# denyingmxd/CFPNet

Measured on AMD Instinct MI355X. Metric: depth maps/sec @ 480x640 bf16 (whole job; per_gpu = value / n_gpus); abs_rel vs CPU oracle, higher is better.
Workload: dtype bf16; 1 GPU; batch=8 480x640 RGB + 8x8-zone ToF, eval forward incl. the prob output [B,256,H/2,W/2] written in the storage dtype (bf16: 2 bytes/element); layers=hist2image combine1 image x2 (CFPNet), parallelism=single GPU

## Files before the change

cfpnet_amd/engine.py:

```python
from __future__ import annotations

import math
import os
from typing import Dict, List, Optional, Sequence, Tuple

import torch

from . import hip, ops, spec
from .geometry import FUSION_SCALES, FusionGeometry, gsa_keys, static_zone_key, zone_records as _zone_records
from .ops import Act

_BN_EPS = 1e-5


def _same_pad(size: int, k: int, s: int) -> Tuple[int, int]:
    total = max((math.ceil(size / s) - 1) * s + k - size, 0)
    return total // 2, total - total // 2


_STREAMS: Dict = {}
_CONCURRENT: Dict[str, list] = {}


def concurrent_streams(device, want: int = 4, pool: int = 16) -> list:
# ... 33 lines not shown
    key = (str(torch.device(device)), role)
    st = _STREAMS.get(key)
    if st is None:
        if isinstance(role, tuple) and role[0] == "lane":
            conc = concurrent_streams(device)
            st = conc[role[1] % len(conc)]
        else:
            st = torch.cuda.Stream(device=device)
        _STREAMS[key] = st
    return st


class Engine:
    def __init__(self, state_dict: Dict[str, torch.Tensor], *, layer_names: Sequence[str], n_bins: int = 256,
                 min_val: float = 1e-3, max_val: float = 10.0, norm: str = "linear", change_embedding: bool = True,
                 no_skip_inside: bool = False, stem_act: bool = False, dtype=None, device="cuda:0",
                 zone_sample_num: int = 16, base_resolution=spec.BASE_RESOLUTION, x3: Optional[bool] = None):
        if dtype is None:
            dtype, x3 = torch.float32, (True if x3 is None else x3)
        x3 = bool(x3)
        hip.load()
        self.base_resolution = tuple(base_resolution)
        self.fusion = spec.fusion_table(self.base_resolution)
        if not torch.cuda.is_available():
            raise RuntimeError("cfpnet_amd.Engine needs a GPU: the product path has no CPU fallback")
        assert dtype in (torch.bfloat16, torch.float16, torch.float32)
        self.layer_names = list(layer_names)
        self.n_bins, self.min_val, self.max_val = n_bins, float(min_val), float(max_val)
        self.norm = {"linear": 0, "softmax": 1, "sigmoid": 2}[norm]
        self.change_embedding, self.no_skip_inside, self.stem_act = change_embedding, no_skip_inside, stem_act
        self.dtype, self.device = dtype, torch.device(device)
        assert not x3 or dtype == torch.float32, "x3 is a matrix-math mode of float32 storage"
        self.x3 = bool(x3)
        self.cdt = hip.F32X3 if self.x3 else ops.DT[dtype]
        self.tickets = self.x3 and os.environ.get("CFP_SPLITK_TICKETS", "0") == "1"
        self.zone_sample_num = zone_sample_num
        self.weights2 = os.environ.get("CFP_WEIGHTS2", "0") == "1"
        self.diffuse_cin = os.environ.get("CFP_DIFFUSE_CIN", "1") == "1"
        self.mbconv_fused = os.environ.get("CFP_MBCONV_FUSED", "0") == "1"
        self.se2 = dtype in (torch.bfloat16, torch.float16) and os.environ.get("CFP_SE2", "1") == "1"
        self.se2_x3 = os.environ.get("CFP_SE2_X3", "1") if self.x3 else "0"
        self._dbg_round = {}
        for item in filter(None, os.environ.get("CFP_DEBUG_ROUND", "").split(",")):
            n, d = item.split(":")
            self._dbg_round[n] = {"f16": torch.float16, "bf16": torch.bfloat16}[d]
        self.up_fused = os.environ.get("CFP_UP_FUSED", "4")
        self.up_fused_x3 = os.environ.get("CFP_UP_FUSED_X3", "")
        self.cat_pad = os.environ.get("CFP_CAT_PAD", "1") == "1" and not self.up_fused_x3
        self.lkpm_fused = os.environ.get("CFP_LKPM_FUSED", "1") != "0"
        self.tail_q = os.environ.get("CFP_TAIL_Q", "1") == "1"
        self.lkpm_min_rows = int(os.environ.get("CFP_LKPM_MIN_ROWS", "30000"))
        self.sr_ln_fused = os.environ.get("CFP_SR_LN_FUSED", "1") == "1"
        self.head_fused = os.environ.get("CFP_HEAD_FUSED", "1") != "0"
        self.er_fused = os.environ.get("CFP_ER_FUSED", "12")
        hl = os.environ.get("CFP_HEAD_HILO", "00")
        self.head_hilo = (hl[0] == "1", hl[1] == "1")
        self.half = dtype in (torch.bfloat16, torch.float16)
        self.ve = 8 if self.half else 4
        self.P: Dict[str, torch.Tensor] = {}
        self._plans: Dict[tuple, dict] = {}
        self._graph = None
        self._splitk_ws: Optional[torch.Tensor] = None
        self._capturing = False
        self._side = _shared_stream(self.device, "side")
        self._lane = 0
        self.use_side_stream = os.environ.get("CFP_NO_SIDE_STREAM", "0") != "1"
        self._lane_streams: Dict[int, Tuple[torch.cuda.Stream, torch.cuda.Stream]] = {}
        self._lanes_active = 1
        self._slots = None
        self._slot_next = 0
        self._lane_ws: Dict[int, torch.Tensor] = {}
        self.load_state_dict(state_dict)

    def _dev(self, t: torch.Tensor, dtype=None) -> torch.Tensor:
        return t.detach().to(device=self.device, dtype=dtype or torch.float32).contiguous()

    def _pack_conv(self, w: torch.Tensor, w2: bool = False) -> torch.Tensor:
        w = w.detach().float()
        if w.dim() == 2:
            w = w[:, :, None, None]
        elif w.dim() == 3:
            w = w[:, :, :, None]
        co, ci, kh, kw = w.shape
        if kh * kw > 1:
            w = ops.round_taps(w, self.dtype)
        cip = (ci + 7) // 8 * 8
        if cip != ci:
            w = torch.nn.functional.pad(w, (0, 0, 0, 0, 0, cip - ci))
        flat = w.permute(0, 2, 3, 1).reshape(co, kh * kw * cip)
        if w2 and self.weights2 and self.half and kh * kw == 1:
            return ops.pack_w2(flat, self.dtype).to(self.device)
        if kh * kw == 1 and self.diffuse_cin and self.dtype == torch.float16:
            flat = ops.round_taps(flat.reshape(co, 1, kh * kw * cip), self.dtype).reshape(co, -1)
        if self.x3:
            return ops.pack_w_x3(self._dev(flat))
        return self._dev(flat, self.dtype)

    def _fold_bn(self, sd, bn: Optional[str], bias: Optional[torch.Tensor], co: int, eps: float):
        if bn is None:
            scale = torch.ones(co)
            shift = bias.detach().float().clone() if bias is not None else torch.zeros(co)
        else:
            g, b = sd[bn + ".weight"].float(), sd[bn + ".bias"].float()
            m, v = sd[bn + ".running_mean"].float(), sd[bn + ".running_var"].float()
            scale = g / torch.sqrt(v + eps)
            shift = b - m * scale
# ... 858 lines not shown
            M = B * hd * wd
            t1 = self._act(plan, f"up{i}.a", M, c[i])
            fits = hd > 1 and wd > 1 and B * hd * wd * cat[i].ld * 2 < 2 ** 31 - 65536 and hs_ * ws_ * src.ld * 2 < 2 ** 31 - 65536
            if self.x3 and str(i) in self.up_fused_x3 and src.C % 32 == 0 and taps is None and hd > 1 and wd > 1:
                n = f"decoder.up{i}.a"
                ops.upsample_cat_conv3x3(src, hs_, ws_, cat[i].slice(src.C, e[i]), self.P[n + ".wcat"], self.P[n + ".s"], self.P[n + ".t"],
                                         t1, B, hd, wd, hip.ACT_LRELU, x3=True)
            elif self.half and str(i) in self.up_fused and src.C % 64 == 0 and taps is None and fits:
                n = f"decoder.up{i}.a"
                ops.upsample_cat_conv3x3(src, hs_, ws_, cat[i].slice(src.C, e[i]), self.P[n + ".w"], self.P[n + ".s"], self.P[n + ".t"],
                                         t1, B, hd, wd, hip.ACT_LRELU)
            else:
                ops.resize_bilinear(src, hs_, ws_, (0, 0, hs_, ws_), cat[i].slice(0, src.C), hd, wd, (0, 0, hd, wd), B)
                n = f"decoder.up{i}.a"
                if (n + ".wpad") in self.P and M >= 30000:
                    ops.conv2d(cat[i], self.P[n + ".wpad"], self.P[n + ".s"], self.P[n + ".t"], t1, B, hd, wd, 3, 3, 1, 1, 1, hd, wd, hip.ACT_LRELU,
                               None, self._ws(M, t1.C, 9 * cat[i].C))
                else:
                    self._cv(n, cat[i].slice(0, src.C + e[i]), t1, B, hd, wd, 3, act=hip.ACT_LRELU)
            if first_only:
                return t1
            t2 = self._act(plan, f"up{i}.b", M, c[i])
            self._cv(f"decoder.up{i}.b", t1, t2, B, hd, wd, 3, act=hip.ACT_LRELU)
            return t2

        main.wait_stream(side)
        xd4 = self._act(plan, "xd4", B * hs[4] * wsz[4], c[0])
        self._cv("decoder.conv4", b4, xd4, B, hs[4], wsz[4], 1)
        x = xd4
        ph, pw = hs[4], wsz[4]
        for i, (fname, feat) in enumerate((("cross_atten3", hfeat[2]), ("cross_atten2", hfeat[1]), ("cross_atten1", hfeat[0])), start=1):
            hh, ww = hs[4 - i], wsz[4 - i]
            D = c[i + 1]
            dcat = self._act(plan, f"dcat{i}", B * hh * ww, 2 * D)
            n3, n1 = f"decoder.up{i}.b", f"decoder.conv{4 - i}"
            if (i == 3 and self.half and (n1 + ".wp") in self.P and "d" in self.er_fused and taps is None
                    and ops.conv3x3_pw_fused_variant(c[i], c[i], D, 1, ops.DT[self.dtype]) >= 0):
                t1 = up(i, x, ph, pw, hh, ww, first_only=True)
                ops.conv3x3_pw_fused(t1, self.P[n3 + ".w"], self.P[n3 + ".s"], self.P[n3 + ".t"], hip.ACT_LRELU, self.P[n1 + ".wp"],
                                     self.P[n1 + ".s"], self.P[n1 + ".t"], dcat.slice(0, D), B, hh, ww, 1, 1, 1, hh, ww)
            else:
                t = up(i, x, ph, pw, hh, ww)
                if taps is not None:
                    taps[f"up{i}"] = self._nchw(t, B, hh, ww)
                self._cv(n1, t, dcat.slice(0, D), B, hh, ww, 1)
            fuse(fname, dcat.slice(0, D), feat, hh, ww, dcat.slice(D, D))
            if taps is not None:
                taps[f"conv{4 - i}"] = self._nchw(dcat.slice(0, D), B, hh, ww)
                taps[fname] = self._nchw(dcat.slice(D, D), B, hh, ww)
            x, ph, pw = dcat, hh, ww
        t = up(4, x, ph, pw, hs[0], wsz[0])
        Mh = B * hs[0] * wsz[0]
        HWh = hs[0] * wsz[0]
        unet = self._act(plan, "unet", Mh, 128)
        fused_head = self.half and self.head_fused and self.n_bins == 256 and HWh % 16 == 0 and HWh >= 128 and "conv_out.wp" in self.P
        ram = self._act(plan, "ram", Mh, 128) if (not fused_head or taps is not None) else None
        edges = out[0] if out is not None else torch.empty(B, self.n_bins + 1, dtype=torch.float32, device=dev)
        centers = self._f32(plan, "head.centers", B * self.n_bins)
        h = "depth_head"
        ns = max(1, min(64, HWh // 256))
        bsum = self._f32(plan, "head.bsum", B * ns * t.C)
        msum = self._f32(plan, "head.msum", B * 128)
        if os.environ.get("CFP_OLD_SUMS", "0") == "1":
            self._cv("decoder.conv0", t, unet, B, hs[0], wsz[0], 3)
        side.wait_stream(main)
        with torch.cuda.stream(side):
            ops.channel_sum(t, bsum, B, HWh, ns)
            ops.conv3x3_mean(bsum, ns, t, self.P["decoder.conv0.w32"], self.P["decoder.conv0.b32"], msum, B, hs[0], wsz[0], 128)
            ops.bin_regressor(msum, 1, 1.0 / HWh, self.P[h + ".w1x1"], self.P[h + ".r0.w"], self.P[h + ".r0.b"], self.P[h + ".r2.w"],
                              self.P[h + ".r2.b"], self.P[h + ".r4.w"], self.P[h + ".r4.b"], self.min_val, self.max_val, self.norm,
                              edges, centers, B, 128, 256, self.n_bins)
        if os.environ.get("CFP_OLD_SUMS", "0") != "1":
            self._cv("decoder.conv0", t, unet, B, hs[0], wsz[0], 3)
        if not fused_head:
            self._cv("depth_head.conv3x3", unet, ram, B, hs[0], wsz[0], 3)
        main.wait_stream(side)
        pred = out[1] if out is not None else torch.empty(B, 1, hs[0], wsz[0], dtype=torch.float32, device=dev)
        if out is not None:
            prob = out[2] if return_prob else None
        else:
            prob = torch.empty(B, self.n_bins, hs[0], wsz[0], dtype=self.dtype, device=dev) if return_prob else None
        unc = None
        if uncertainty:
            unc = out[3] if out is not None else torch.empty(B, 3, hs[0], wsz[0], dtype=torch.float32, device=dev)
        if fused_head:
            ops.depth_head_fused(unet, self.P[h + ".conv3x3.w"], self.P[h + ".conv3x3.s"], self.P[h + ".conv3x3.t"], self.P["conv_out.wp"],
                                 self.P["conv_out.t"], centers, prob, pred, B, hs[0], wsz[0], ram_out=ram, ram_hilo=self.head_hilo[1],
                                 stats=unc)
        elif (self.half or self.x3) and self.n_bins == 256 and HWh % 8 == 0 and os.environ.get("CFP_BIN_HEAD_FUSED", "1") != "0":
            ops.bin_head_fused(ram, self.P["conv_out.w"], self.P["conv_out.t"], centers, prob, pred, B, HWh, stats=unc)
        else:
            logits = self._act(plan, "logits", Mh, self.n_bins)
            self._lin("conv_out.w", ram, logits, Mh, hip.ACT_NONE, None, "conv_out")
            ops.bin_softmax(logits, centers, prob, pred, B, HWh, self.n_bins, stats=unc)
        if taps is not None:
            taps["unet_out"] = self._nchw(unet, B, hs[0], wsz[0])
            taps["ram"] = self._nchw(ram, B, hs[0], wsz[0])
        return (edges, pred, prob, unc) if uncertainty else (edges, pred, prob)
```

cfpnet_amd/hip.py:

```python
from __future__ import annotations

import ctypes as C
import os
from typing import Optional

_HERE = os.path.dirname(os.path.abspath(__file__))
LIB_PATH = os.environ.get("CFP_HIP_LIB") or os.path.join(_HERE, "libcfpnet_hip.so")

F32, BF16, F16 = 0, 1, 2
F32X3 = 3
ACT_NONE, ACT_RELU, ACT_LRELU, ACT_SILU, ACT_GELU, ACT_SIGMOID = range(6)
TOF_SAMPLE_UNIFORM, TOF_SAMPLE_ICDF = 0, 1
HEAD_WOUT_HILO, HEAD_RAM_HILO = 1, 2
UNC_STD, UNC_ENTROPY, UNC_PMAX = 0, 1, 2
SPARS_STD, SPARS_ENTROPY, SPARS_PMAX, SPARS_ORACLE_RMSE, SPARS_ORACLE_ABSREL = range(5)
REGION_ALL, REGION_FOV_IN, REGION_FOV_OUT, REGION_ZONE_VALID, REGION_ZONE_INVALID = range(5)
CONV_PER_IMAGE, CONV_W2, CONV_IN_FLIGHT, CONV_X3, CONV_WS_TICKETS = 1, 2, 4, 8, 16
CONV_TICKET_BYTES = 4096

_p, _i, _f, _sz, _ll = C.c_void_p, C.c_int, C.c_float, C.c_size_t, C.c_longlong

SIGNATURES = {
    "cfp_version": (_i, []),
    "cfp_last_error": (C.c_char_p, []),
# ... 80 lines not shown
    "cfp_bn_train_bwd": (_i, [_p, _i, _p, _i, C.c_longlong, _i, _i, _p, _p, _p, _p, _i, _p, _p, _p, _i, _p, _sz, _p]),
    "cfp_colsum": (_i, [_p, _i, C.c_longlong, _i, _i, _p, _p, _sz, _p]),
    "cfp_act_bwd": (_i, [_p, _i, _p, _i, _i, _p, _i, C.c_longlong, _i, _i, _p]),
    "cfp_layernorm_bwd_ws_bytes": (_sz, [C.c_longlong, _i]),
    "cfp_layernorm_bwd": (_i, [_p, _i, _p, _i, _p, _f, _p, _i, _i, _p, _p, C.c_longlong, _i, _i, _p, _sz, _p]),
    "cfp_layernorm_bwd_deferred": (_i, [_p, _i, _p, _i, _p, _f, _p, _i, _i, _p, _p, C.c_longlong, _i, _i, _p, _sz, _p, _p]),
    "cfp_axpby": (_i, [_p, _i, _p, _i, _f, _f, _p, _i, C.c_longlong, _i, _i, _p]),
    "cfp_rowtable_grad": (_i, [_p, _i, _p, _i, _i, _i, _i, _i, _i, _i, _f, _i, _p]),
    "cfp_se_train_ws_floats": (_sz, [_i, _i, _i]),
    "cfp_se_train_fwd": (_i, [_p, _i, _f] + [_p] * 7 + [_i, _i, _i, _p]),
    "cfp_se_train_bwd": (_i, [_p] * 12 + [_f, _f, _i, _i, _i, _p]),
    "cfp_channel_dot": (_i, [_p, _i, _p, _i, _p, _i, _i, _i, _i, _p]),
    "cfp_bcast_fma": (_i, [_p, _i, _p, _p, _p, _i, _i, _i, _i, _i, _p]),
    "cfp_dwconv3x3_dgrad": (_i, [_p, _i, _p, _p, _i] + [_i] * 11 + [_p]),
    "cfp_dwconv3x3_wgrad_ws_bytes": (_sz, [_i]),
    "cfp_dwconv3x3_wgrad": (_i, [_p, _i, _p, _i, _p] + [_i] * 9 + [_f, _i, _p, _sz, _p]),
    "cfp_dwconv3x3_wgrad_deferred": (_i, [_p, _i, _p, _i, _p] + [_i] * 9 + [_f, _i, _p, _sz, _p, _p]),
    "cfp_index_rows": (_i, [_p, _i, _p, _p, _i, C.c_longlong, _i, _i, _i, _p]),
    "cfp_resize_bilinear_bwd": (_i, [_p, _i, _p, _i, _i, _i, _i, _i, _i, _i, _i, _i, _p]),
    "cfp_bin_centers": (_i, [_p, _f, _f, _p, _p, _i, _i, _p]),
    "cfp_bin_centers_bwd": (_i, [_p, _f, _f, _p, _i, _i, _p]),
    "cfp_softmax_expect_ws_bytes": (_sz, [_i, _i, _i]),
    "cfp_softmax_expect": (_i, [_p, _i, _p, _p, _p, _p, _i, _p, _i, _i, _i, _i, _p, _sz, _p]),
    "cfp_linattn_state_bytes": (_sz, [_i, _i, _i]),
    "cfp_linattn_ws_bytes": (_sz, [_i, _i, _i, _i, _i]),
    "cfp_linattn_fwd": (_i, [_p, _i, _p, _i, _p, _i, _p, _i, _p, _i, _i, _i, _i, _i, _f, _i, _p, _sz, _p]),
    "cfp_linattn_bwd": (_i, [_p, _i, _p, _i, _p, _i, _p, _i, _p, _p, _i, _p, _i, _p, _i, _i, _i, _i, _i, _i, _f, _i, _p, _sz, _p]),
    "cfp_linattn_fwd_dev": (_i, [_p, _i, _p, _i, _p, _i, _p, _i, _p, _i, _i, _i, _i, _i, _f, _i, _p, _sz, _p, _p]),
    "cfp_linattn_bwd_dev": (_i, [_p, _i, _p, _i, _p, _i, _p, _i, _p, _p, _i, _p, _i, _p, _i, _i, _i, _i, _i, _i, _f, _i, _p, _sz, _p, _p]),
    "cfp_zone_crop": (_i, [_p, _i, _p, _p, _i] + [_i] * 7 + [_i, _p]),
    "cfp_zone_crop_bwd": (_i, [_p, _i, _p, _p, _i] + [_i] * 7 + [_i, _p]),
    "cfp_zone_paste": (_i, [_p, _i, _p, _i, _p, _p, _i] + [_i] * 7 + [_i, _p]),
    "cfp_zone_paste_bwd": (_i, [_p, _i, _p, _p, _i] + [_i] * 7 + [_i, _p]),
    "cfp_zone_rect_rows": (_i, [_p, _i, _p, _p, _i] + [_i] * 6 + [_i, _p]),
    "cfp_dwconv_large_wgrad_ws_bytes": (_sz, [_i, _i, _i, _i, _i]),
    "cfp_dwconv_large_wgrad": (_i, [_p, _i, _p, _i, _p, _i, _i, _i, _i, _i, _f, _i, _p, _sz, _p]),
    "cfp_row_normalize": (_i, [_p, _p, _p, _i, _i, _p]),
    "cfp_add_rowtable_dev": (_i, [_p, _i, _p, _p, _i, _i, _i, _i, _i, _i, _i, _p, _i, _p]),
    "cfp_rowtable_grad_dev": (_i, [_p, _i, _p, _i, _i, _i, _i, _i, _i, _p, _f, _i, _p]),
    "cfp_nyu_augment": (_i, [_p, _p, _i, _i, _i, _p, _p, _p, _i, _i, C.POINTER(C.c_float), C.POINTER(C.c_float), _p, _p, _p]),
    "cfp_nyu_rotate": (_i, [_p, _p, _p, _p, _i, _i, _i, _p, _p]),
    "cfp_bin_regressor": (_i, [_p, _i, _f] + [_p] * 7 + [_f, _f, _i, _p, _p, _i, _i, _i, _i, _p]),
    "cfp_bin_softmax": (_i, [_p, _i, _p, _p, _p, _i, _i, _i, _i, _p]),
    "cfp_bin_softmax_stats": (_i, [_p, _i, _p, _p, _p, _p, _i, _i, _i, _i, _p]),
    "cfp_conv3x3_mean": (_i, [_p, _i, _p, _i, _p, _p, _p, _i, _i, _i, _i, _i, _i, _p]),
    "cfp_lkpm_tail": (_i, [_p, _i, _p, _i, _p, _i, _p, _p, _p, _p, _p, _p, _f, _i, _i, _i, _p]),
    "cfp_mbconv_plan": (_i, [_i, _i, _i, _i, _i, _p, _p]),
    "cfp_mbconv_expand_dw": (_i, [_p, _i, _p, _p, _p, _p, _p, _p, _p, _i, _p, _i, _i, _i, _i, _i, _i, _p]),
    "cfp_conv3x3_pw_fused_variant": (_i, [_i] * 5),
    "cfp_conv3x3_pw_fused": (_i, [_p, _i, _p, _p, _p, _i, _p, _p, _p, _i, _p, _i, _p, _i] + [_i] * 12 + [_p]),
    "cfp_hist_encoder": (_i, [_p, _p, _p, _p, _p, _p, _p, _p, _p, _i, _i, _i, _p]),
    "cfp_depth_head_fused": (_i, [_p, _i, _p, _p, _p, _p, _p, _p, _p, _p, _p, _i, _i, _i, _i, _i, _p]),
    "cfp_bin_head_fused": (_i, [_p, _i, _p, _p, _p, _p, _p, _i, _i, _i, _i, _p]),
    "cfp_depth_head_fused_stats": (_i, [_p, _i, _p, _p, _p, _p, _p, _p, _p, _p, _p, _p, _i, _i, _i, _i, _i, _p]),
    "cfp_bin_head_fused_stats": (_i, [_p, _i, _p, _p, _p, _p, _p, _p, _i, _i, _i, _i, _p]),
}

class WgradJob(C.Structure):
    _fields_ = [("slabs", C.c_void_p), ("dw", C.c_void_p), ("db", C.c_void_p), ("n", C.c_longlong), ("n_dw", C.c_longlong),
                ("nsplit", C.c_int), ("ew", C.c_int), ("beta", C.c_float), ("beta_b", C.c_float)]


_lib: Optional[C.CDLL] = None


def load() -> C.CDLL:
    global _lib
    if _lib is not None:
        return _lib
    if not os.path.exists(LIB_PATH):
        raise RuntimeError(
            f"{LIB_PATH} not found: build the HIP extension first "
            f"(`python -c 'import __graft_entry__ as g; g.build()'` or `make -C cfpnet_amd/csrc`). "
            "There is no CPU fallback for the product path.")
    import torch
    lib = C.CDLL(LIB_PATH)
    for name, (res, args) in SIGNATURES.items():
        fn = getattr(lib, name)
        fn.restype = res
        fn.argtypes = args
    _lib = lib
    return lib


def last_error() -> str:
    return load().cfp_last_error().decode()


def call(name: str, *args):
    rc = getattr(load(), name)(*args)
    if rc != 0:
        raise RuntimeError(f"{name} failed ({rc}): {last_error()}")


def ptr(t) -> int:
    return 0 if t is None else t.data_ptr()


def current_stream() -> int:
    import torch
    return torch.cuda.current_stream().cuda_stream
```

cfpnet_amd/ops.py:

```python
from __future__ import annotations

import os
from dataclasses import dataclass
from typing import Optional, Tuple

import torch

from . import hip

DT = {torch.float32: hip.F32, torch.bfloat16: hip.BF16, torch.float16: hip.F16}


@dataclass
class Act:
    buf: torch.Tensor
    c0: int
    C: int

    @property
    def rows(self) -> int:
        return self.buf.shape[0]

    @property
    def ld(self) -> int:
# ... 453 lines not shown
    wp = w[:, src]
    hi = (round_taps(w.reshape(256, 1, 128), dtype).reshape(256, 128)[:, src] if diffuse else wp).to(dtype)
    planes = [hi]
    if hilo:
        planes.append((wp - hi.float()).to(dtype))
    return torch.stack(planes).contiguous()


def pw_k_order(K: int) -> torch.Tensor:
    pos = torch.arange((K + 31) // 32 * 32)
    kb, q, e = pos // 32, (pos % 32) // 8, pos % 8
    src = 32 * kb + 16 * (e // 4) + 4 * q + (e % 4)
    return torch.where(src < K, src, torch.full_like(src, -1))


def pad_pw_w(w: torch.Tensor) -> torch.Tensor:
    co, K = w.shape
    out = torch.zeros((co + 15) // 16 * 16, (K + 31) // 32 * 32, dtype=w.dtype, device=w.device)
    out[:co, :K] = w
    return out.contiguous()


def conv3x3_pw_fused_variant(Cin: int, Cmid: int, Cout: int, stride: int, dt: int) -> int:
    return int(hip.load().cfp_conv3x3_pw_fused_variant(Cin, Cmid, Cout, stride, dt))


def conv3x3_pw_fused(x: Act, w1: torch.Tensor, s1, t1, act1, w2_pad: torch.Tensor, s2, t2, out: Act, B, H, W, stride, pad_t, pad_l, Ho, Wo,
                     act2=hip.ACT_NONE, residual: Optional[Act] = None):
    mid = w1.shape[0]
    assert x.rows >= B * H * W and out.rows >= B * Ho * Wo and x.dt == out.dt
    assert w1.dtype == x.buf.dtype and tuple(w1.shape) == (mid, 9 * x.C) and w1.is_contiguous()
    assert w2_pad.dtype == x.buf.dtype and tuple(w2_pad.shape) == ((out.C + 15) // 16 * 16, (mid + 31) // 32 * 32) and w2_pad.is_contiguous()
    hip.call("cfp_conv3x3_pw_fused", x.ptr, x.ld, w1.data_ptr(), hip.ptr(s1), hip.ptr(t1), act1, w2_pad.data_ptr(), hip.ptr(s2), hip.ptr(t2), act2,
             residual.ptr if residual else 0, residual.ld if residual else 0, out.ptr, out.ld, B, H, W, x.C, mid, out.C, stride, pad_t, pad_l,
             Ho, Wo, x.dt, _s())


def depth_head_fused(x: Act, w3, scale3, shift3, wout_perm: torch.Tensor, bias_out, centers, prob, pred, B, H, W, ram_out: Optional[Act] = None,
                     ram_hilo: bool = True, probe: int = 0, stats=None):
    assert x.C == 128 and w3.shape == (128, 9 * 128) and wout_perm.shape[1:] == (256, 128) and wout_perm.dtype == x.buf.dtype
    flags = (hip.HEAD_WOUT_HILO if wout_perm.shape[0] == 2 else 0) | (hip.HEAD_RAM_HILO if ram_hilo else 0) | (probe << 8)
    if ram_out is not None:
        assert ram_out.ld == 128 and ram_out.C == 128
    if stats is None:
        hip.call("cfp_depth_head_fused", x.ptr, x.ld, w3.data_ptr(), hip.ptr(scale3), hip.ptr(shift3), wout_perm.data_ptr(), bias_out.data_ptr(),
                 centers.data_ptr(), hip.ptr(prob), pred.data_ptr(), ram_out.ptr if ram_out is not None else 0, B, H, W, flags, x.dt, _s())
        return
    _check_stats(stats, B, H * W)
    hip.call("cfp_depth_head_fused_stats", x.ptr, x.ld, w3.data_ptr(), hip.ptr(scale3), hip.ptr(shift3), wout_perm.data_ptr(), bias_out.data_ptr(),
             centers.data_ptr(), hip.ptr(prob), pred.data_ptr(), stats.data_ptr(), ram_out.ptr if ram_out is not None else 0, B, H, W, flags,
             x.dt, _s())


def hist_encoder(hist: torch.Tensor, blob: torch.Tensor, layout, outs, R: int, pe=(None, None, None), n_pe: int = 0):
    import ctypes
    assert hist.dtype == torch.float32 and hist.is_contiguous() and hist.numel() >= R and blob.dtype == torch.float32 and len(layout) == 9
    flat = [int(v) for row in layout for v in row]
    arr = (ctypes.c_int * len(flat))(*flat)
    for o, row in zip(outs, layout[2::3]):
        assert o.C == row[4] and o.ld == o.C and o.c0 == 0 and o.rows >= R
    for t, o in zip(pe, outs):
        assert t is None or (t.dtype == torch.float32 and tuple(t.shape) == (n_pe, o.C) and t.is_contiguous())
    hip.call("cfp_hist_encoder", hist.data_ptr(), blob.data_ptr(), ctypes.addressof(arr), outs[0].ptr, outs[1].ptr, outs[2].ptr,
             hip.ptr(pe[0]), hip.ptr(pe[1]), hip.ptr(pe[2]), n_pe, R, outs[0].dt, _s())


def conv3x3_mean(partial: torch.Tensor, nsplit, x: Act, w32: torch.Tensor, bias, msum: torch.Tensor, B, H, W, Cout):
    assert w32.dtype == torch.float32 and tuple(w32.shape) == (Cout, 9 * x.C) and msum.dtype == torch.float32 and msum.numel() >= B * Cout
    hip.call("cfp_conv3x3_mean", partial.data_ptr(), nsplit, x.ptr, x.ld, w32.data_ptr(), hip.ptr(bias), msum.data_ptr(), B, H, W, x.C, Cout, x.dt, _s())


def mbconv_plan(B, H, W, Cin, mid):
    import ctypes
    t, kp = ctypes.c_int(0), ctypes.c_int(0)
    rc = hip.load().cfp_mbconv_plan(B, H, W, Cin, mid, ctypes.byref(t), ctypes.byref(kp))
    return (t.value, kp.value) if rc == 0 else None


def pack_mbconv_pw(w2d: torch.Tensor, dtype) -> torch.Tensor:
    mid, cin = w2d.shape
    kp = (cin + 31) // 32 * 32
    out = torch.zeros(mid, kp + 8, dtype=dtype)
    out[:, :cin] = w2d.to(dtype)
    return out.contiguous()


def mbconv_expand_dw(x: Act, wpw: torch.Tensor, s1, t1, wdw: torch.Tensor, s2, t2, out: Act, partial: Optional[torch.Tensor], B, H, W):
    mid = out.C
    assert wpw.dtype == x.buf.dtype and wpw.shape[0] == mid and wdw.shape == (9, mid) and wdw.dtype == x.buf.dtype
    hip.call("cfp_mbconv_expand_dw", x.ptr, x.ld, wpw.data_ptr(), s1.data_ptr(), t1.data_ptr(), wdw.data_ptr(), s2.data_ptr(), t2.data_ptr(),
             out.ptr, out.ld, hip.ptr(partial), B, H, W, x.C, mid, x.dt, _s())


def lkpm_tail(t: Act, xin: Act, out: Act, w1, b1, w2, b2, ln_g, ln_b, rows, ln_eps=1e-6):
    D = t.C
    x3 = t.buf.dtype == torch.float32 and w1.dtype == torch.float16
    k1, k2 = (2 * D, 8 * D) if x3 else (D, 4 * D)
    assert xin.C == D and out.C == D and tuple(w1.shape) == (4 * D, k1) and tuple(w2.shape) == (D, k2) and (x3 or w1.dtype == t.buf.dtype)
    hip.call("cfp_lkpm_tail", t.ptr, t.ld, xin.ptr, xin.ld, out.ptr, out.ld, w1.data_ptr(), b1.data_ptr(), w2.data_ptr(), b2.data_ptr(),
             ln_g.data_ptr(), ln_b.data_ptr(), float(ln_eps), rows, D, hip.F32X3 if x3 else t.dt, _s())
```

include/cfpnet_hip.h:

```cpp
#ifndef CFPNET_HIP_H
#define CFPNET_HIP_H

#include <stddef.h>
#include <stdint.h>

#ifdef __cplusplus
extern "C" {
#endif

typedef void* cfp_stream_t;

enum { CFP_OK = 0, CFP_EINVAL = -1, CFP_ESHAPE = -2, CFP_EHIP = -3 };
enum { CFP_F32 = 0, CFP_BF16 = 1, CFP_F16 = 2 };
enum { CFP_F32X3 = 3 };
enum { CFP_TOF_SAMPLE_UNIFORM = 0, CFP_TOF_SAMPLE_ICDF = 1 };
enum { CFP_ACT_NONE = 0, CFP_ACT_RELU = 1, CFP_ACT_LRELU = 2, CFP_ACT_SILU = 3, CFP_ACT_GELU = 4, CFP_ACT_SIGMOID = 5 };

int cfp_version(void);
const char* cfp_last_error(void);

int cfp_conv2d_nhwc(const void* in, int in_ld, const void* w, const float* scale, const float* shift,
                    const void* residual, int res_ld, void* out, int out_ld,
                    int B, int H, int W, int Cin, int Cout, int KH, int KW, int stride,
                    int pad_t, int pad_l, int Ho, int Wo, int act, int dtype,
// ... 107 lines not shown
int cfp_resize_bilinear(const void* src, int src_ld, int Hs, int Ws, int sy0, int sx0, int sh, int sw,
                        void* dst, int dst_ld, int Hd, int Wd, int dy0, int dx0, int dh, int dw,
                        const uint8_t* zone_valid, int zn, int p1, int p2, int accumulate,
                        int B, int C, int dtype, cfp_stream_t stream);

int cfp_resize_bilinear_dev(const void* src, int src_ld, int Hs, int Ws, void* dst, int dst_ld, int Hd, int Wd,
                            const int* rec, int rec_side, const uint8_t* zone_valid, int zn, int p1, int p2,
                            int accumulate, int B, int C, int dtype, cfp_stream_t stream);

int cfp_add_rowtable(const void* in, int in_ld, const float* table, void* out, int out_ld, int rows, int C,
                     int H, int W, int Wt, int oy, int ox, int dtype, cfp_stream_t stream);

int cfp_upsample_cat_conv3x3(const void* low, int low_ld, int Hs, int Ws, int Cup, const void* skip, int skip_ld, int Cskip,
                             const void* w, const float* scale, const float* shift, void* out, int out_ld, int B, int H, int W,
                             int Cout, int act, int dtype, cfp_stream_t stream);

int cfp_copy_rows(const void* in, int in_ld, void* out, int out_ld, int rows, int C, int dtype, cfp_stream_t stream);
int cfp_copy_rows2(const void* in0, int in0_ld, void* out0, int out0_ld, int C0, const void* in1, int in1_ld, void* out1, int out1_ld,
                   int C1, int rows, int dtype, cfp_stream_t stream);

int cfp_rgb_to_nhwc8(const float* rgb, void* out, int B, int H, int W, int dtype, cfp_stream_t stream);
int cfp_rgb_to_nhwc8_hilo(const float* rgb, void* out, int B, int H, int W, int dtype, cfp_stream_t stream);
int cfp_scalar_to_rows8(const float* in, void* out, int rows, int dtype, cfp_stream_t stream);

int cfp_hist_encoder(const float* hist, const float* blob, const int* layout, void* out0, void* out1, void* out2,
                     const float* pe0, const float* pe1, const float* pe2, int n_pe, int R, int dtype, cfp_stream_t stream);

int cfp_lkpm_tail(const void* t, int t_ld, const void* xin, int x_ld, void* out, int out_ld, const void* w1, const float* b1,
                  const void* w2, const float* b2, const float* ln_g, const float* ln_b, float ln_eps, int rows, int D, int dtype,
                  cfp_stream_t stream);

int cfp_bin_regressor(const float* partial, int nsplit, float inv_hw, const float* w1x1_t,
                      const float* w0_t, const float* b0, const float* w1_t, const float* b1,
                      const float* w2_t, const float* b2, float min_val, float max_val, int norm,
                      float* edges, float* centers, int B, int C, int hidden, int nbins, cfp_stream_t stream);

int cfp_conv3x3_mean(const float* partial, int nsplit, const void* in, int in_ld, const float* w, const float* bias, float* msum,
                     int B, int H, int W, int C, int Cout, int dtype, cfp_stream_t stream);

int cfp_bin_softmax(const void* logits, int ld, const float* centers, void* prob, float* pred,
                    int B, int HW, int nbins, int dtype, cfp_stream_t stream);

enum { CFP_UNC_STD = 0, CFP_UNC_ENTROPY = 1, CFP_UNC_PMAX = 2 };
int cfp_bin_softmax_stats(const void* logits, int ld, const float* centers, void* prob, float* pred, float* stats,
                          int B, int HW, int nbins, int dtype, cfp_stream_t stream);

enum { CFP_HEAD_WOUT_HILO = 1, CFP_HEAD_RAM_HILO = 2 };
int cfp_depth_head_fused(const void* x, int x_ld, const void* w3, const float* scale3, const float* shift3,
                         const void* wout_perm, const float* bias_out, const float* centers, void* prob, float* pred,
                         void* ram_out, int B, int H, int W, int flags, int dtype, cfp_stream_t stream);
int cfp_depth_head_fused_stats(const void* x, int x_ld, const void* w3, const float* scale3, const float* shift3,
                               const void* wout_perm, const float* bias_out, const float* centers, void* prob, float* pred,
                               float* stats, void* ram_out, int B, int H, int W, int flags, int dtype, cfp_stream_t stream);

int cfp_bin_head_fused(const void* x, int x_ld, const void* w, const float* bias, const float* centers,
                       void* prob, float* pred, int B, int HW, int Cin, int dtype, cfp_stream_t stream);
int cfp_bin_head_fused_stats(const void* x, int x_ld, const void* w, const float* bias, const float* centers,
                             void* prob, float* pred, float* stats, int B, int HW, int Cin, int dtype, cfp_stream_t stream);


size_t cfp_silog_ws_bytes(int B, int Ht, int Wt);
int cfp_silog_loss_fwd(const float* pred, int Hp, int Wp, const float* target, const unsigned char* mask, int Ht, int Wt,
                       int B, int interpolate, void* ws, size_t ws_bytes, float* stats, cfp_stream_t stream);
int cfp_silog_loss_bwd(const void* ws, const float* stats, float grad_loss, int Hp, int Wp, int Ht, int Wt, int B,
                       int interpolate, float* grad_pred, cfp_stream_t stream);

int cfp_adamw_step(float* param, const float* grad, float* exp_avg, float* exp_avg_sq, long long n, float lr,
                   float beta1, float beta2, float eps, float weight_decay, int step, const float* grad_scale,
                   cfp_stream_t stream);
size_t cfp_grad_clip_ws_bytes(void);
int cfp_grad_clip_factor(const float* grad, long long n, float max_norm, void* ws, size_t ws_bytes, float* out,
                         cfp_stream_t stream);


int cfp_tof_hist_sim(const float* depth, long long img_stride, int B, int H, int W, int zone_num, int zone_px, int sy0,
                     int sx0, const int* offsets, int offset_bound, float max_distance, int bins, double bin_width,
                     int floor_count, const float* w0, const float* w1, int nsamp, int sample_mode, double* fh, float* rect,
                     unsigned char* mask, float* pts, int* hist_out, cfp_stream_t stream);
int cfp_tof_sample_points(const double* fh, const unsigned char* mask, const float* w0, const float* w1, long long nzones,
                          int nsamp, int sample_mode, float* pts, cfp_stream_t stream);

size_t cfp_eval_metrics_ws_bytes(int B);
int cfp_eval_metrics(const float* pred, int Hp, int Wp, const float* gt, int H, int W, int B, int interpolate, int mode,
                     float lo, float hi, void* ws, size_t ws_bytes, double* out, cfp_stream_t stream);

enum { CFP_SPARS_STD = 0, CFP_SPARS_ENTROPY, CFP_SPARS_PMAX, CFP_SPARS_ORACLE_RMSE, CFP_SPARS_ORACLE_ABSREL };
size_t cfp_unc_sparsification_ws_bytes(int B, int H, int W, int steps);
int cfp_unc_sparsification(const float* pred, const float* unc, int Hp, int Wp, const float* gt, int H, int W, int B,
                           int interpolate, int mode, float lo, float hi, int steps, void* ws, size_t ws_bytes,
                           double* curves , double* summary ,
                           double* n_valid , cfp_stream_t stream);

enum { CFP_REGION_ALL = 0, CFP_REGION_FOV_IN, CFP_REGION_FOV_OUT, CFP_REGION_ZONE_VALID, CFP_REGION_ZONE_INVALID };
size_t cfp_eval_metrics_regions_ws_bytes(int B);
int cfp_eval_metrics_regions(const float* pred, int Hp, int Wp, const float* gt, int H, int W, int B, int interpolate, int mode,
                             float lo, float hi, const float* rect , const unsigned char* mask , int Z,
                             const float* edges , int n_edges, void* ws, size_t ws_bytes,
                             double* out , cfp_stream_t stream);

int cfp_depth_unproject(const float* pred, int Hp, int Wp, int H, int W, int B, int interpolate, float lo, float hi,
                        const float* K , float* points ,
                        float* normals , cfp_stream_t stream);

size_t cfp_points_compact_ws_bytes(int B, int H, int W, int stride);
int cfp_points_compact(const float* points, const float* normals, int H, int W, int B, int stride, float z_near, float z_far,
                       const float* unc, int Hu, int Wu, long long unc_stride, float unc_lo, float unc_hi, int cap,
// ... 154 lines not shown
```

Measured before the change: 3823 maps/s.

## Fuse decoder.conv0 into the depth head kernel with halo recompute

Adds a single HIP kernel that computes decoder.conv0 (3x3, 32->128) on an 18x18 halo tile in LDS, then runs the depth head 3x3 conv, the 1x1 bin logits, softmax, prob write and pred. It is enabled by default when the shape fits. This removes the round trip of the 128-channel unet activation through HBM and one kernel launch. In exchange it recomputes halo pixels, needs about 160 KB of LDS per workgroup (one block per CU), and rounds the intermediate to bf16 inside the kernel.

```diff
diff --git a/cfpnet_amd/csrc/head_conv0.hip b/cfpnet_amd/csrc/head_conv0.hip
--- /dev/null
+++ b/cfpnet_amd/csrc/head_conv0.hip
@@ -0,0 +1,387 @@
+#include "common.h"
+
+namespace {
+
+typedef __attribute__((address_space(3))) void* lds_ptr_t;
+
+constexpr int HC_C = 128;
+constexpr int HC_NB = 256;
+constexpr int HC_CIN = 32;
+constexpr int HC_K0 = 9 * HC_CIN;
+constexpr int HC_K3 = 9 * HC_C;
+constexpr int HC_STEPS = HC_K3 / 64;
+constexpr int HC_WSTAGE = HC_C * 128;
+constexpr int HC_TW = 20, HC_TPIX = HC_TW * HC_TW, HC_TP = 80;
+constexpr int HC_UW = 18, HC_UPIX = HC_UW * HC_UW, HC_UP = 288;
+constexpr int HC_UGROUPS = (HC_UPIX + 15) / 16;
+constexpr int HC_OFF_T = 2 * HC_WSTAGE;
+constexpr int HC_OFF_U = 65536;
+constexpr int HC_OFF_K = HC_OFF_U + HC_UPIX * HC_UP;
+constexpr int HC_LDS = HC_OFF_K + 4 * 256 * 4;
+constexpr int HC_BM = 256;
+constexpr int HC_PPITCH = HC_BM + 8;
+constexpr unsigned HC_OOB = 0x80000000u;
+static_assert(HC_OFF_T + HC_TPIX * HC_TP <= HC_OFF_U, "t halo");
+static_assert(HC_NB * HC_PPITCH * 2 <= HC_OFF_K, "prob staging must end before the constants");
+static_assert(HC_LDS <= 160 * 1024, "LDS of a CU");
+
+struct HeadC0P {
+  const void* t; const void* w0; const float* scale0; const float* shift0;
+  const void* w3; const float* scale3; const float* shift3;
+  const void* wout; const float* bias_out; const float* centers;
+  void* prob; float* pred;
+  int t_ld, B, H, W, HW, tiles_x, tiles_y;
+  int probe;
+};
+
+__device__ __forceinline__ void hc_handover() {
+  asm volatile("s_waitcnt vmcnt(0) lgkmcnt(0)" ::: "memory");
+  __syncthreads();
+  asm volatile("" ::: "memory");
+}
+
+template <typename H>
+__global__ __launch_bounds__(512, 1) void depth_head_conv0_kernel(HeadC0P p) {
+  extern __shared__ __attribute__((aligned(16))) unsigned char smem[];
+  unsigned char* sT = smem + HC_OFF_T;
+  unsigned char* sU = smem + HC_OFF_U;
+  float* sK = reinterpret_cast<float*>(smem + HC_OFF_K);
+  const int tid = threadIdx.x;
+  const int lane = tid & 63;
+  const int wave = __builtin_amdgcn_readfirstlane(tid >> 6);
+  const int fr = lane & 15, fq = lane >> 4;
+  const int rsub = lane >> 3;
+  const int lc = (lane & 7) ^ rsub;
+  int bid = xcd_remap(blockIdx.x, gridDim.x);
+  const int x0 = (bid % p.tiles_x) * 16; bid /= p.tiles_x;
+  const int y0 = (bid % p.tiles_y) * 16;
+  const int b = bid / p.tiles_y;
+
+  const int live = (p.probe & 1) ? 0 : 1;
+  const auto rs_t = __builtin_amdgcn_make_buffer_rsrc((void*)p.t, 0, (int)((unsigned)p.B * (unsigned)p.HW * (unsigned)p.t_ld * 2u) * live, 0x00020000);
+  const auto rs_w0 = __builtin_amdgcn_make_buffer_rsrc((void*)p.w0, 0, HC_C * HC_K0 * 2 * live, 0x00020000);
+  const auto rs_w3 = __builtin_amdgcn_make_buffer_rsrc((void*)p.w3, 0, HC_C * HC_K3 * 2 * live, 0x00020000);
+  const auto rs_o = __builtin_amdgcn_make_buffer_rsrc((void*)p.wout, 0, HC_NB * HC_C * 2 * live, 0x00020000);
+
+  auto issue_w0 = [&](int ks, int buf) {
+#pragma unroll
+    for (int i = 0; i < 2; ++i) {
+      const int g = i * 8 + wave;
+      const unsigned v = (ks * 8 + lc) * 8 < HC_K0 ? (unsigned)(g * 8 + rsub) * (unsigned)(HC_K0 * 2) + (unsigned)lc * 16u : HC_OOB;
+      __builtin_amdgcn_raw_ptr_buffer_load_lds(rs_w0, (lds_ptr_t)(smem + buf * HC_WSTAGE + g * 1024), 16, (int)v, ks * 128, 0, 0);
+    }
+  };
+  auto issue_w3 = [&](int ks, int buf) {
+#pragma unroll
+    for (int i = 0; i < 2; ++i) {
+      const int g = i * 8 + wave;
+      const unsigned v = (unsigned)(g * 8 + rsub) * (unsigned)(HC_K3 * 2) + (unsigned)lc * 16u;
+      __builtin_amdgcn_raw_ptr_buffer_load_lds(rs_w3, (lds_ptr_t)(smem + buf * HC_WSTAGE + g * 1024), 16, (int)v, ks * 128, 0, 0);
+    }
+  };
+  auto issue_wout = [&](int half, int off) {
+#pragma unroll
+    for (int q = 0; q < 4; ++q) {
+      const int g = q * 8 + wave;
+      const unsigned v = (unsigned)(g * 8 + rsub) * (unsigned)(HC_C * 2) + (unsigned)lc * 16u;
+      __builtin_amdgcn_raw_ptr_buffer_load_lds(rs_o, (lds_ptr_t)(smem + off + g * 1024), 16, (int)v, half * 128, 0, 0);
+    }
+  };
+
+  issue_w0(0, 0);
+
+  {
+    u32x4 v[4];
+    int dst[4];
+#pragma unroll
+    for (int n = 0; n < 4; ++n) {
+      const int i = tid + n * 512;
+      const int px = i >> 2, ch = i & 3;
+      const int hy = px / HC_TW, hx = px - hy * HC_TW;
+      const int y = y0 - 2 + hy, x = x0 - 2 + hx;
+      const bool ok = px < HC_TPIX && (unsigned)y < (unsigned)p.H && (unsigned)x < (unsigned)p.W;
+      const unsigned off = ok ? (unsigned)((b * p.H + y) * p.W + x) * (unsigned)p.t_ld * 2u + (unsigned)ch * 16u : HC_OOB;
+      v[n] = __builtin_amdgcn_raw_buffer_load_b128(rs_t, (int)off, 0, 0);
+      dst[n] = px < HC_TPIX ? px * HC_TP + ch * 16 : -1;
+    }
+    if (tid < 256) {
+      sK[tid] = p.bias_out[tid];
+      sK[512 + tid] = p.centers[(long long)b * HC_NB + tid];
+    } else if (tid < 384) {
+      const int u = tid - 256;
+      sK[256 + u] = p.scale3 ? p.scale3[u] : 1.f;
+      sK[768 + u] = p.scale0 ? p.scale0[u] : 1.f;
+    } else {
+      const int u = tid - 384;
+      sK[384 + u] = p.shift3 ? p.shift3[u] : 0.f;
+      sK[896 + u] = p.shift0 ? p.shift0[u] : 0.f;
+    }
+#pragma unroll
+    for (int n = 0; n < 4; ++n)
+      if (dst[n] >= 0) *reinterpret_cast<u32x4*>(sT + dst[n]) = v[n];
+  }
+
+  {
+    const int ng = wave + 16 < HC_UGROUPS ? 3 : 2;
+    int tb[3];
+#pragma unroll
+    for (int g = 0; g < 3; ++g) {
+      const int q = min((wave + 8 * g) * 16 + fr, HC_UPIX - 1);
+      const int hy = q / HC_UW, hx = q - hy * HC_UW;
+      tb[g] = (hy * HC_TW + hx) * HC_TP + fq * 16;
+    }
+    f32x4 acc0[3][8];
+#pragma unroll
+    for (int g = 0; g < 3; ++g)
+#pragma unroll
+      for (int i = 0; i < 8; ++i) acc0[g][i] = f32x4{0.f, 0.f, 0.f, 0.f};
+#pragma unroll
+    for (int ks = 0; ks < 5; ++ks) {
+      hc_handover();
+      if (ks < 4) issue_w0(ks + 1, (ks + 1) & 1);
+      else issue_w3(0, 1);
+      const unsigned char* cW = smem + (ks & 1) * HC_WSTAGE;
+#pragma unroll
+      for (int s = 0; s < 2; ++s) {
+        const int tap = 2 * ks + s;
+        if (tap >= 9) break;
+        const int pc = ((s * 4 + fq) ^ (fr & 7)) * 16;
+        const int toff = ((tap / 3) * HC_TW + tap % 3) * HC_TP;
+        s16x8 wf[8], xf[3];
+#pragma unroll
+        for (int i = 0; i < 8; ++i) wf[i] = *reinterpret_cast<const s16x8*>(cW + (i * 16 + fr) * 128 + pc);
+#pragma unroll
+        for (int g = 0; g < 3; ++g)
+          if (g < ng) xf[g] = *reinterpret_cast<const s16x8*>(sT + tb[g] + toff);
+#pragma unroll
+        for (int g = 0; g < 3; ++g)
+          if (g < ng) {
+#pragma unroll
+            for (int i = 0; i < 8; ++i) acc0[g][i] = mfma16<H>(wf[i], xf[g], acc0[g][i]);
+          }
+      }
+    }
+#pragma unroll
+    for (int g = 0; g < 3; ++g) {
+      if (g >= ng) continue;
+      const int q = (wave + 8 * g) * 16 + fr;
+      const int hy = q / HC_UW, hx = q - hy * HC_UW;
+      const int y = y0 - 1 + hy, x = x0 - 1 + hx;
+      const bool inside = (unsigned)y < (unsigned)p.H && (unsigned)x < (unsigned)p.W;
+#pragma unroll
+      for (int i = 0; i < 8; ++i) {
+        const int ch = i * 16 + fq * 4;
+        float sc[4], sh[4], yv[4];
+        Vec<float>::load(sK + 768 + ch, sc);
+        Vec<float>::load(sK + 896 + ch, sh);
+#pragma unroll
+        for (int r = 0; r < 4; ++r) yv[r] = acc0[g][i][r] * sc[r] + sh[r];
+        uint2 pk;
+        pk.x = inside ? pack2<H>(yv[0], yv[1]) : 0u;
+        pk.y = inside ? pack2<H>(yv[2], yv[3]) : 0u;
+        if (q < HC_UPIX) *reinterpret_cast<uint2*>(sU + q * HC_UP + ch * 2) = pk;
+      }
+    }
+  }
+  if (p.probe & 8) {
+    asm volatile("s_waitcnt vmcnt(0) lgkmcnt(0)" ::: "memory");
+    return;
+  }
+
+  f32x4 acc1[8][2];
+#pragma unroll
+  for (int i = 0; i < 8; ++i)
+#pragma unroll
+    for (int j = 0; j < 2; ++j) acc1[i][j] = f32x4{0.f, 0.f, 0.f, 0.f};
+  const unsigned char* urow = sU + ((2 * wave) * HC_UW + fr) * HC_UP + fq * 16;
+  for (int ks = 0; ks < HC_STEPS; ++ks) {
+    hc_handover();
+    if (ks == 0) issue_wout(0, HC_OFF_T);
+    if (ks + 1 < HC_STEPS) issue_w3(ks + 1, ks & 1);
+    const int tap = ks >> 1;
+    const int dy = tap / 3, dx = tap - dy * 3;
+    const unsigned char* cP = urow + (dy * HC_UW + dx) * HC_UP + (ks & 1) * 128;
+    const unsigned char* cW = smem + ((ks + 1) & 1) * HC_WSTAGE;
+#pragma unroll
+    for (int s = 0; s < 2; ++s) {
+      const int pc = ((s * 4 + fq) ^ (fr & 7)) * 16;
+      s16x8 wf[8], pf[2];
+#pragma unroll
+      for (int j = 0; j < 2; ++j) pf[j] = *reinterpret_cast<const s16x8*>(cP + j * (HC_UW * HC_UP) + s * 64);
+#pragma unroll
+      for (int i = 0; i < 8; ++i) wf[i] = *reinterpret_cast<const s16x8*>(cW + (i * 16 + fr) * 128 + pc);
+#pragma unroll
+      for (int i = 0; i < 8; ++i)
+#pragma unroll
+        for (int j = 0; j < 2; ++j) acc1[i][j] = mfma16<H>(wf[i], pf[j], acc1[i][j]);
+    }
+  }
+  hc_handover();
+  issue_wout(1, 0);
+  if (p.probe & 2) {
+    asm volatile("s_waitcnt vmcnt(0)" ::: "memory");
+    if (tid == 0 && acc1[0][0][0] == 123.456f) p.pred[0] = acc1[7][1][3];
+    return;
+  }
+
+  s16x8 bh[4][2];
+#pragma unroll
+  for (int kb = 0; kb < 4; ++kb) {
+    float sc[2][4], sh[2][4];
+#pragma unroll
+    for (int u = 0; u < 2; ++u) {
+      const int ch = (2 * kb + u) * 16 + fq * 4;
+      Vec<float>::load(sK + 256 + ch, sc[u]);
+      Vec<float>::load(sK + 384 + ch, sh[u]);
+    }
+#pragma unroll
+    for (int j = 0; j < 2; ++j) {
+      float v[8];
+#pragma unroll
+      for (int u = 0; u < 2; ++u)
+#pragma unroll
+        for (int r = 0; r < 4; ++r) v[u * 4 + r] = acc1[2 * kb + u][j][r] * sc[u][r] + sh[u][r];
+      uint32_t hi[4];
+#pragma unroll
+      for (int e = 0; e < 4; ++e) {
+        const H h0 = from_f32<H>(v[2 * e]), h1 = from_f32<H>(v[2 * e + 1]);
+        hi[e] = (uint32_t)to_bits<H>(h0) | ((uint32_t)to_bits<H>(h1) << 16);
+      }
+      bh[kb][j] = __builtin_bit_cast(s16x8, u32x4{hi[0], hi[1], hi[2], hi[3]});
+    }
+  }
+
+  __builtin_amdgcn_sched_barrier(0);
+
+  f32x4 acc2[16][2];
+#pragma unroll
+  for (int ti = 0; ti < 16; ++ti) {
+    float b4[4];
+    Vec<float>::load(sK + ti * 16 + fq * 4, b4);
+#pragma unroll
+    for (int j = 0; j < 2; ++j) acc2[ti][j] = f32x4{b4[0], b4[1], b4[2], b4[3]};
+  }
+  auto gemm2_half = [&](int half, const unsigned char* base) {
+#pragma unroll
+    for (int kl = 0; kl < 2; ++kl) {
+      const int kb = half * 2 + kl;
+      const int pc = ((kl * 4 + fq) ^ (fr & 7)) * 16;
+#pragma unroll
+      for (int ti = 0; ti < 16; ++ti) {
+        const s16x8 af = *reinterpret_cast<const s16x8*>(base + (ti * 16 + fr) * 128 + pc);
+#pragma unroll
+        for (int j = 0; j < 2; ++j) acc2[ti][j] = mfma16<H>(af, bh[kb][j], acc2[ti][j]);
+      }
+    }
+  };
+  gemm2_half(0, smem + HC_OFF_T);
+  hc_handover();
+  gemm2_half(1, smem);
+  if (p.probe & 4) {
+    if (tid == 0 && acc2[0][0][0] == 123.456f) p.pred[0] = acc2[15][1][3];
+    return;
+  }
+  __syncthreads();
+
+  H* sP = reinterpret_cast<H*>(smem);
+  H* prob = reinterpret_cast<H*>(p.prob);
+#pragma unroll
+  for (int j = 0; j < 2; ++j) {
+    const int pl = wave * 32 + j * 16 + fr;
+    float mx = -3.0e38f;
+#pragma unroll
+    for (int ti = 0; ti < 16; ++ti)
+#pragma unroll
+      for (int r = 0; r < 4; ++r) mx = fmaxf(mx, acc2[ti][j][r]);
+    mx = fmaxf(mx, __shfl_xor(mx, 16, 64));
+    mx = fmaxf(mx, __shfl_xor(mx, 32, 64));
+    float s = 0.f;
+#pragma unroll
+    for (int ti = 0; ti < 16; ++ti)
+#pragma unroll
+      for (int r = 0; r < 4; ++r) {
+        const float d = acc2[ti][j][r] - mx;
+        const float e = __expf(d);
+        acc2[ti][j][r] = e;
+        s += e;
+      }
+    s += __shfl_xor(s, 16, 64);
+    s += __shfl_xor(s, 32, 64);
+    const float inv = 1.f / s;
+    float dot = 0.f;
+#pragma unroll
+    for (int ti = 0; ti < 16; ++ti) {
+      float cen[4];
+      Vec<float>::load(sK + 512 + ti * 16 + fq * 4, cen);
+#pragma unroll
+      for (int r = 0; r < 4; ++r) {
+        const float pr = acc2[ti][j][r] * inv;
+        dot = fmaf(pr, cen[r], dot);
+        if (prob) sP[(ti * 16 + fq * 4 + r) * HC_PPITCH + pl] = from_f32<H>(pr);
+      }
+    }
+    dot += __shfl_xor(dot, 16, 64);
+    dot += __shfl_xor(dot, 32, 64);
+    if (fq == 0) p.pred[(long long)b * p.HW + (y0 + 2 * wave + j) * p.W + x0 + fr] = dot;
+  }
+  if (!prob) return;
+  __syncthreads();
+#pragma unroll 4
+  for (int q = tid; q < HC_NB * 32; q += 512) {
+    const int n = q >> 5, c = q & 31;
+    const int row = c >> 1, half = c & 1;
+    *reinterpret_cast<u32x4*>(prob + ((long long)b * HC_NB + n) * p.HW + (y0 + row) * p.W + x0 + half * 8) =
+        *reinterpret_cast<const u32x4*>(sP + n * HC_PPITCH + row * 16 + half * 8);
+  }
+}
+
+}
+
+extern "C" int cfp_depth_head_conv0_fused(const void* t, int t_ld, const void* w0, const float* scale0, const float* shift0, const void* w3,
+                                          const float* scale3, const float* shift3, const void* wout_perm, const float* bias_out,
+                                          const float* centers, void* prob, float* pred, int B, int H, int W, int flags, int dtype,
+                                          cfp_stream_t stream) {
+  CFP_REQUIRE(is16(dtype), CFP_EINVAL, "cfp_depth_head_conv0_fused: bf16/f16 only");
+  CFP_REQUIRE(t && w0 && w3 && wout_perm && bias_out && centers && pred, CFP_EINVAL, "cfp_depth_head_conv0_fused: null pointer");
+  CFP_REQUIRE(B > 0 && H > 0 && W > 0 && t_ld >= HC_CIN && t_ld % 8 == 0, CFP_ESHAPE, "cfp_depth_head_conv0_fused: bad shape (32 input channels, t_ld % 8 == 0)");
+  CFP_REQUIRE(H % 16 == 0 && W % 16 == 0, CFP_ESHAPE, "cfp_depth_head_conv0_fused: H and W must be multiples of the 16 x 16 tile");
+  const long long M = (long long)B * H * W;
+  CFP_REQUIRE(M * t_ld * 2 < (1ll << 31) - 4096 && M / 256 < (1ll << 31), CFP_ESHAPE, "cfp_depth_head_conv0_fused: input larger than 2 GB");
+  CFP_REQUIRE(aligned16(t) && aligned16(w0) && aligned16(w3) && aligned16(wout_perm) && aligned16(prob) && aligned16(bias_out) && aligned16(centers) &&
+                  aligned16(scale0) && aligned16(shift0) && aligned16(scale3) && aligned16(shift3), CFP_EINVAL,
+              "cfp_depth_head_conv0_fused: pointers must be 16-byte aligned");
+  CFP_REQUIRE((flags & ~(15 << 8)) == 0, CFP_EINVAL, "cfp_depth_head_conv0_fused: unknown flags");
+  static int lds_max = -1;
+  if (lds_max < 0) {
+    int dev = 0, v = 0;
+    if (hipGetDevice(&dev) != hipSuccess || hipDeviceGetAttribute(&v, hipDeviceAttributeMaxSharedMemoryPerBlock, dev) != hipSuccess) {
+      cfp_set_error("cfp_depth_head_conv0_fused: cannot query the LDS size");
+      return CFP_EHIP;
+    }
+    lds_max = v;
+  }
+  CFP_REQUIRE(lds_max >= HC_LDS, CFP_ESHAPE, "cfp_depth_head_conv0_fused: the device does not grant 162944 bytes of LDS to a workgroup");
+  HeadC0P p;
+  p.t = t; p.w0 = w0; p.scale0 = scale0; p.shift0 = shift0; p.w3 = w3; p.scale3 = scale3; p.shift3 = shift3;
+  p.wout = wout_perm; p.bias_out = bias_out; p.centers = centers; p.prob = prob; p.pred = pred;
+  p.t_ld = t_ld; p.B = B; p.H = H; p.W = W; p.HW = H * W; p.tiles_x = W / 16; p.tiles_y = H / 16;
+  p.probe = (flags >> 8) & 15;
+  const int grid = (int)(M / HC_BM);
+  hipStream_t s = reinterpret_cast<hipStream_t>(stream);
+#define HC_LAUNCH(T)                                                                                                                       \
+  do {                                                                                                                                     \
+    static bool attr = false;                                                                                                              \
+    if (!attr) {                                                                                                                           \
+      if (hipFuncSetAttribute((const void*)depth_head_conv0_kernel<T>, hipFuncAttributeMaxDynamicSharedMemorySize, HC_LDS) != hipSuccess) { \
+        cfp_set_error("cfp_depth_head_conv0_fused: cannot set the LDS size");                                                              \
+        return CFP_EHIP;                                                                                                                   \
+      }                                                                                                                                    \
+      attr = true;                                                                                                                         \
+    }                                                                                                                                      \
+    hipLaunchKernelGGL((depth_head_conv0_kernel<T>), dim3(grid), dim3(512), HC_LDS, s, p);                                                 \
+  } while (0)
+  if (dtype == CFP_F16) HC_LAUNCH(f16_t);
+  else HC_LAUNCH(bf16_t);
+#undef HC_LAUNCH
+  return cfp_check_launch("cfp_depth_head_conv0_fused");
+}
diff --git a/cfpnet_amd/engine.py b/cfpnet_amd/engine.py
--- a/cfpnet_amd/engine.py
+++ b/cfpnet_amd/engine.py
@@ -109,6 +109,7 @@
         self.lkpm_min_rows = int(os.environ.get("CFP_LKPM_MIN_ROWS", "30000"))
         self.sr_ln_fused = os.environ.get("CFP_SR_LN_FUSED", "1") == "1"
         self.head_fused = os.environ.get("CFP_HEAD_FUSED", "1") != "0"
+        self.head_conv0 = os.environ.get("CFP_HEAD_CONV0", "1") != "0"
         self.er_fused = os.environ.get("CFP_ER_FUSED", "12")
         hl = os.environ.get("CFP_HEAD_HILO", "00")
         self.head_hilo = (hl[0] == "1", hl[1] == "1")
@@ -1073,8 +1074,10 @@
         t = up(4, x, ph, pw, hs[0], wsz[0])
         Mh = B * hs[0] * wsz[0]
         HWh = hs[0] * wsz[0]
-        unet = self._act(plan, "unet", Mh, 128)
         fused_head = self.half and self.head_fused and self.n_bins == 256 and HWh % 16 == 0 and HWh >= 128 and "conv_out.wp" in self.P
+        head_conv0 = (fused_head and self.head_conv0 and taps is None and not uncertainty and self.head_hilo == (False, False)
+                      and os.environ.get("CFP_OLD_SUMS", "0") != "1" and t.C == 32 and ops.depth_head_conv0_fits(hs[0], wsz[0]))
+        unet = None if head_conv0 else self._act(plan, "unet", Mh, 128)
         ram = self._act(plan, "ram", Mh, 128) if (not fused_head or taps is not None) else None
         edges = out[0] if out is not None else torch.empty(B, self.n_bins + 1, dtype=torch.float32, device=dev)
         centers = self._f32(plan, "head.centers", B * self.n_bins)
@@ -1091,7 +1094,7 @@
             ops.bin_regressor(msum, 1, 1.0 / HWh, self.P[h + ".w1x1"], self.P[h + ".r0.w"], self.P[h + ".r0.b"], self.P[h + ".r2.w"],
                               self.P[h + ".r2.b"], self.P[h + ".r4.w"], self.P[h + ".r4.b"], self.min_val, self.max_val, self.norm,
                               edges, centers, B, 128, 256, self.n_bins)
-        if os.environ.get("CFP_OLD_SUMS", "0") != "1":
+        if os.environ.get("CFP_OLD_SUMS", "0") != "1" and not head_conv0:
             self._cv("decoder.conv0", t, unet, B, hs[0], wsz[0], 3)
         if not fused_head:
             self._cv("depth_head.conv3x3", unet, ram, B, hs[0], wsz[0], 3)
@@ -1104,7 +1107,11 @@
         unc = None
         if uncertainty:
             unc = out[3] if out is not None else torch.empty(B, 3, hs[0], wsz[0], dtype=torch.float32, device=dev)
-        if fused_head:
+        if head_conv0:
+            ops.depth_head_conv0_fused(t, self.P["decoder.conv0.w"], self.P["decoder.conv0.s"], self.P["decoder.conv0.t"], self.P[h + ".conv3x3.w"],
+                                       self.P[h + ".conv3x3.s"], self.P[h + ".conv3x3.t"], self.P["conv_out.wp"], self.P["conv_out.t"], centers,
+                                       prob, pred, B, hs[0], wsz[0])
+        elif fused_head:
             ops.depth_head_fused(unet, self.P[h + ".conv3x3.w"], self.P[h + ".conv3x3.s"], self.P[h + ".conv3x3.t"], self.P["conv_out.wp"],
                                  self.P["conv_out.t"], centers, prob, pred, B, hs[0], wsz[0], ram_out=ram, ram_hilo=self.head_hilo[1],
                                  stats=unc)
diff --git a/cfpnet_amd/hip.py b/cfpnet_amd/hip.py
--- a/cfpnet_amd/hip.py
+++ b/cfpnet_amd/hip.py
@@ -156,6 +156,7 @@
     "cfp_hist_encoder": (_i, [_p, _p, _p, _p, _p, _p, _p, _p, _p, _i, _i, _i, _p]),
     "cfp_depth_head_fused": (_i, [_p, _i, _p, _p, _p, _p, _p, _p, _p, _p, _p, _i, _i, _i, _i, _i, _p]),
     "cfp_bin_head_fused": (_i, [_p, _i, _p, _p, _p, _p, _p, _i, _i, _i, _i, _p]),
+    "cfp_depth_head_conv0_fused": (_i, [_p, _i, _p, _p, _p, _p, _p, _p, _p, _p, _p, _p, _p, _i, _i, _i, _i, _i, _p]),
     "cfp_depth_head_fused_stats": (_i, [_p, _i, _p, _p, _p, _p, _p, _p, _p, _p, _p, _p, _i, _i, _i, _i, _i, _p]),
     "cfp_bin_head_fused_stats": (_i, [_p, _i, _p, _p, _p, _p, _p, _p, _i, _i, _i, _i, _p]),
 }
diff --git a/cfpnet_amd/ops.py b/cfpnet_amd/ops.py
--- a/cfpnet_amd/ops.py
+++ b/cfpnet_amd/ops.py
@@ -529,6 +529,19 @@
              x.dt, _s())
 
 
+def depth_head_conv0_fits(H: int, W: int) -> bool:
+    return H % 16 == 0 and W % 16 == 0
+
+
+def depth_head_conv0_fused(t: Act, w0, scale0, shift0, w3, scale3, shift3, wout_perm: torch.Tensor, bias_out, centers, prob, pred, B, H, W,
+                           probe: int = 0):
+    assert t.C == 32 and t.rows >= B * H * W and tuple(w0.shape) == (128, 9 * 32) and tuple(w3.shape) == (128, 9 * 128)
+    assert tuple(wout_perm.shape) == (1, 256, 128) and wout_perm.dtype == t.buf.dtype and w0.dtype == t.buf.dtype and w3.dtype == t.buf.dtype
+    hip.call("cfp_depth_head_conv0_fused", t.ptr, t.ld, w0.data_ptr(), hip.ptr(scale0), hip.ptr(shift0), w3.data_ptr(), hip.ptr(scale3),
+             hip.ptr(shift3), wout_perm.data_ptr(), bias_out.data_ptr(), centers.data_ptr(), hip.ptr(prob), pred.data_ptr(), B, H, W,
+             probe << 8, t.dt, _s())
+
+
 def hist_encoder(hist: torch.Tensor, blob: torch.Tensor, layout, outs, R: int, pe=(None, None, None), n_pe: int = 0):
     import ctypes
     assert hist.dtype == torch.float32 and hist.is_contiguous() and hist.numel() >= R and blob.dtype == torch.float32 and len(layout) == 9
diff --git a/include/cfpnet_hip.h b/include/cfpnet_hip.h
--- a/include/cfpnet_hip.h
+++ b/include/cfpnet_hip.h
@@ -183,6 +183,11 @@
 int cfp_depth_head_fused_stats(const void* x, int x_ld, const void* w3, const float* scale3, const float* shift3,
                                const void* wout_perm, const float* bias_out, const float* centers, void* prob, float* pred,
                                float* stats, void* ram_out, int B, int H, int W, int flags, int dtype, cfp_stream_t stream);
+
+int cfp_depth_head_conv0_fused(const void* t, int t_ld, const void* w0, const float* scale0, const float* shift0, const void* w3,
+                               const float* scale3, const float* shift3, const void* wout_perm, const float* bias_out,
+                               const float* centers, void* prob, float* pred, int B, int H, int W, int flags, int dtype,
+                               cfp_stream_t stream);
 
 int cfp_bin_head_fused(const void* x, int x_ld, const void* w, const float* bias, const float* centers,
                        void* prob, float* pred, int B, int HW, int Cin, int dtype, cfp_stream_t stream);
```

New measurement: 3911 maps/s, median of 6. 1.02x the previous value.
